# Nightmare-n/GD-MAE

Measured on AMD Instinct MI355X. Metric: MAE pre-train frames/sec (Waymo-shape, 180k pts, 75% mask), higher is better.
Workload: dtype bf16

## Files before the change

gd-mae_amd/csrc/chamfer.hip:

```cpp
#include "common.h"

struct GtParams {
  float lo[3], vs[3];
  int ncols;
  int K;
};

__global__ __launch_bounds__(256) void k_group_gt(const float* __restrict__ pts, const int* __restrict__ pt_off,
                                                  const int* __restrict__ csr, const long long* __restrict__ voxel_coords,
                                                  int M, GtParams P, float* __restrict__ gt, int* __restrict__ gidx) {
  const int lane = threadIdx.x & (GD_WAVE - 1);
  const int wib = threadIdx.x / GD_WAVE;
  for (int p = blockIdx.x * 4 + wib; p < M; p += gridDim.x * 4) {
    const int off = pt_off[p];
    const int cnt = pt_off[p + 1] - off;
    const long long* vc = voxel_coords + 4ll * p;
    const float cx = __fadd_rn(__fmul_rn(__fadd_rn((float)vc[3], 0.5f), P.vs[0]), P.lo[0]);
    const float cy = __fadd_rn(__fmul_rn(__fadd_rn((float)vc[2], 0.5f), P.vs[1]), P.lo[1]);
    const float cz = __fadd_rn(__fmul_rn(__fadd_rn((float)vc[1], 0.5f), P.vs[2]), P.lo[2]);
    for (int k = lane; k < P.K; k += GD_WAVE) {
      const int src = k < cnt ? k : k % cnt;
      const int pid = csr[off + src];
      const float* r = pts + (long long)pid * P.ncols;
      float* o = gt + ((long long)p * P.K + k) * 3;
// ... 25 lines not shown
}

template <int P1MAX>
__global__ __launch_bounds__(256) void k_chamfer(const float* __restrict__ pred, const float* __restrict__ gt,
                                                 const float* __restrict__ w, int M, int P1, int P2,
                                                 float* __restrict__ term, float* __restrict__ dpred) {
  __shared__ float sx[4][P1MAX * 3];
  const int lane = threadIdx.x & (GD_WAVE - 1);
  const int wib = threadIdx.x / GD_WAVE;
  for (int m = blockIdx.x * 4 + wib; m < M; m += gridDim.x * 4) {
    const float wm = w[m];
    float* dp = dpred + (long long)m * P1 * 3;
    if (wm == 0.f) {
      for (int e = lane; e < P1 * 3; e += GD_WAVE) dp[e] = 0.f;
      if (lane == 0) term[m] = 0.f;
      continue;
    }
    for (int e = lane; e < P1 * 3; e += GD_WAVE) sx[wib][e] = pred[(long long)m * P1 * 3 + e];
    __builtin_amdgcn_wave_barrier();
    const bool has = lane < P2;
    float y0 = 0.f, y1 = 0.f, y2 = 0.f;
    if (has) {
      const float* g = gt + ((long long)m * P2 + lane) * 3;
      y0 = g[0];
      y1 = g[1];
      y2 = g[2];
    }
    float best = INFINITY;
    int besti = 0;
    float sumx = 0.f;
    const float cx = wm / (float)P1, cy = wm / (float)P2;
    for (int i = 0; i < P1; ++i) {
      const float x0 = sx[wib][3 * i], x1 = sx[wib][3 * i + 1], x2 = sx[wib][3 * i + 2];
      const float d0 = x0 - y0, d1 = x1 - y1, d2 = x2 - y2;
      const float d = has ? (d0 * d0 + d1 * d1 + d2 * d2) : INFINITY;
      if (d < best) {
        best = d;
        besti = i;
      }
      const float dmin = gd_wave_min(d);
      const unsigned long long bal = __ballot(d == dmin);
      const int jstar = __ffsll((long long)bal) - 1;
      sumx += dmin;
      const float g0 = 2.f * cx * __shfl(d0, jstar, GD_WAVE);
      const float g1 = 2.f * cx * __shfl(d1, jstar, GD_WAVE);
      const float g2 = 2.f * cx * __shfl(d2, jstar, GD_WAVE);
      if (lane == 0) {
        dp[3 * i] = g0;
        dp[3 * i + 1] = g1;
        dp[3 * i + 2] = g2;
      }
    }
    const float sumy = gd_wave_sum(has ? best : 0.f);
    if (lane == 0) term[m] = cx * sumx + cy * sumy;
    __builtin_amdgcn_fence(__ATOMIC_RELEASE, "workgroup");
    for (int i = 0; i < P1; ++i) {
      const bool mine = has && besti == i;
      const float x0 = sx[wib][3 * i], x1 = sx[wib][3 * i + 1], x2 = sx[wib][3 * i + 2];
      const float a0 = gd_wave_sum(mine ? 2.f * cy * (x0 - y0) : 0.f);
      const float a1 = gd_wave_sum(mine ? 2.f * cy * (x1 - y1) : 0.f);
      const float a2 = gd_wave_sum(mine ? 2.f * cy * (x2 - y2) : 0.f);
      if (lane == 0) {
        dp[3 * i] += a0;
        dp[3 * i + 1] += a1;
        dp[3 * i + 2] += a2;
      }
    }
    __builtin_amdgcn_wave_barrier();
  }
}

template <int N>
__device__ __forceinline__ void ch_tstep(unsigned long long (&k)[16], int mask, int lane) {
  const bool hi = (lane & mask) != 0;
#pragma unroll
  for (int t = 0; t < N; ++t) {
    const unsigned long long send = hi ? k[t] : k[t + N];
    const unsigned long long keep = hi ? k[t + N] : k[t];
    const unsigned long long recv = __shfl_xor(send, mask, GD_WAVE);
    k[t] = keep < recv ? keep : recv;
  }
}

__global__ __launch_bounds__(256) void k_chamfer16(const float* __restrict__ pred, const float* __restrict__ gt,
                                                   const float* __restrict__ w, int M, int P2, float* __restrict__ term,
                                                   float* __restrict__ dpred) {
  __shared__ float sx[4][48];
  __shared__ float sy[4][GD_WAVE * 3];
  __shared__ int sb[4][GD_WAVE];
  __shared__ float sg[4][48];
  const int lane = threadIdx.x & (GD_WAVE - 1);
  const int wib = threadIdx.x / GD_WAVE;
  const int my_i = ((lane >> 5) & 1) * 8 + ((lane >> 4) & 1) * 4 + ((lane >> 3) & 1) * 2 + ((lane >> 2) & 1);
  for (int m = blockIdx.x * 4 + wib; m < M; m += gridDim.x * 4) {
    const float wm = w[m];
    float* dp = dpred + (long long)m * 48;
    if (wm == 0.f) {
      if (lane < 48) dp[lane] = 0.f;
      if (lane == 0) term[m] = 0.f;
      continue;
    }
    if (lane < 48) sx[wib][lane] = pred[(long long)m * 48 + lane];
    const bool has = lane < P2;
    float y0 = 0.f, y1 = 0.f, y2 = 0.f;
    if (has) {
      const float* g = gt + ((long long)m * P2 + lane) * 3;
      y0 = g[0];
      y1 = g[1];
      y2 = g[2];
    }
    __builtin_amdgcn_wave_barrier();
    const float cx = wm / 16.f, cy = wm / (float)P2;
    unsigned long long k[16];
    float best = INFINITY;
    int besti = 0;
#pragma unroll
    for (int i = 0; i < 16; ++i) {
      const float d0 = sx[wib][3 * i] - y0, d1 = sx[wib][3 * i + 1] - y1, d2 = sx[wib][3 * i + 2] - y2;
      const float d = has ? (d0 * d0 + d1 * d1 + d2 * d2) : INFINITY;
      if (d < best) {
        best = d;
        besti = i;
      }
      k[i] = ((unsigned long long)__float_as_uint(d) << 32) | (unsigned)lane;
    }
    ch_tstep<8>(k, 32, lane);
    ch_tstep<4>(k, 16, lane);
    ch_tstep<2>(k, 8, lane);
    ch_tstep<1>(k, 4, lane);
    unsigned long long k0 = k[0];
    {
      unsigned long long o = __shfl_xor(k0, 2, GD_WAVE);
      k0 = k0 < o ? k0 : o;
      o = __shfl_xor(k0, 1, GD_WAVE);
      k0 = k0 < o ? k0 : o;
    }
    const float dmin = __uint_as_float((unsigned)(k0 >> 32));
    const int jstar = (int)(k0 & 63u);
    const float ys0 = __shfl(y0, jstar, GD_WAVE), ys1 = __shfl(y1, jstar, GD_WAVE), ys2 = __shfl(y2, jstar, GD_WAVE);
    if ((lane & 3) == 0) {
      sg[wib][3 * my_i] = 2.f * cx * (sx[wib][3 * my_i] - ys0);
      sg[wib][3 * my_i + 1] = 2.f * cx * (sx[wib][3 * my_i + 1] - ys1);
      sg[wib][3 * my_i + 2] = 2.f * cx * (sx[wib][3 * my_i + 2] - ys2);
    }
    const float sumx = gd_wave_sum((lane & 3) == 0 ? dmin : 0.f);
    const float sumy = gd_wave_sum(has ? best : 0.f);
    if (lane == 0) term[m] = cx * sumx + cy * sumy;
    sy[wib][3 * lane] = y0;
    sy[wib][3 * lane + 1] = y1;
    sy[wib][3 * lane + 2] = y2;
    sb[wib][lane] = has ? besti : -1;
    __builtin_amdgcn_fence(__ATOMIC_RELEASE, "workgroup");
    __builtin_amdgcn_wave_barrier();
    if (lane < 48) {
      const int i = lane / 3, c = lane - 3 * i;
      const float xi = sx[wib][lane];
      float acc = 0.f;
      for (int j = 0; j < P2; ++j) {
        const float v = 2.f * cy * (xi - sy[wib][3 * j + c]);
        acc += sb[wib][j] == i ? v : 0.f;
      }
      dp[lane] = sg[wib][lane] + acc;
    }
    __builtin_amdgcn_wave_barrier();
  }
}

extern "C" int gdmae_chamfer(const float* pred, const float* gt, const float* weights, int M, int P1, int P2, float* term,
                             float* dpred, void* stream) {
  if (M <= 0) return 0;
  GD_REQUIRE(P2 >= 1 && P2 <= GD_WAVE, "NUM_GT_POINTS must be <= 64 (one lane per ground-truth point)");
  GD_REQUIRE(P1 >= 1 && P1 <= 64, "NUM_PRD_POINTS must be <= 64");
  int grid = gd_div_up(M, 4);
  if (grid > 8192) grid = 8192;
  if (P1 == 16)
    hipLaunchKernelGGL(k_chamfer16, dim3(grid), dim3(256), 0, (hipStream_t)stream, pred, gt, weights, M, P2, term, dpred);
  else
    hipLaunchKernelGGL((k_chamfer<64>), dim3(grid), dim3(256), 0, (hipStream_t)stream, pred, gt, weights, M, P1, P2, term,
                       dpred);
  GD_LAUNCH_CHECK();
  return 0;
}
```

gd-mae_amd/gdmae_hip/lib.py:

```python
from __future__ import annotations

import ctypes as C
import os

import torch

_HERE = os.path.dirname(os.path.abspath(__file__))
LIB_PATH = os.path.abspath(os.path.join(_HERE, "..", "csrc", "libgdmae_hip.so"))
if os.environ.get("GDMAE_LIB"):
    LIB_PATH = os.path.abspath(os.environ["GDMAE_LIB"])


class GdmaeHipError(RuntimeError):
    pass


_P, _I, _L, _F, _D, _Z = C.c_void_p, C.c_int, C.c_longlong, C.c_float, C.c_double, C.c_size_t

SIGNATURES = {
    "gdmae_abi_version": (_I, []),
    "gdmae_target_arch": (C.c_char_p, []),
    "gdmae_last_error": (C.c_char_p, []),
    "gdmae_voxelize_workspace_bytes": (_Z, [_L, _I, _I, _I, _I]),
    "gdmae_voxelize": (_I, [_P, _L, _I, _P, _P, _P, _I, _P, _P, _P, _P, _P, _P, _P, _P, _P, _P, _P, _P, _P, _P, _Z, _P]),
# ... 59 lines not shown
    "gdmae_window_attention_levels_bwd": (_I, [_P, _P, _P, _P, _P, _I, _P, _P, _P, _P, _I, _P, _P, _I, _I, _P, _F, _P, _P, _P]),
    "gdmae_conv3x3_dense_packed_bytes": (_Z, [_I, _I]),
    "gdmae_conv3x3_dense_pack": (_I, [_P, _I, _I, _I, _I, _P, _P]),
    "gdmae_conv3x3_dense": (_I, [_P, _I, _I, _I, _I, _I, _I, _P, _P, _P, _P]),
    "gdmae_conv3x3_dense_add": (_I, [_P, _I, _I, _I, _I, _I, _I, _P, _P, _P, _P, _P]),
    "gdmae_conv3x3_dense_relu": (_I, [_P, _I, _I, _I, _I, _I, _I, _P, _P, _P, _P, _P]),
    "gdmae_conv3x3_dense_stats_workspace_bytes": (_Z, [_I, _I, _I, _I]),
    "gdmae_conv3x3_dense_stat_rows": (_I, []),
    "gdmae_conv3x3_dense_stats": (_I, [_P, _I, _I, _I, _I, _I, _I, _P, _P, _P, _P, _P, _P]),
    "gdmae_bn_fold_partials": (_I, [_P, _I, _I, _D, _P, _P, _D, _D, _P, _P, _P, _P, _P, _P, _P]),
    "gdmae_conv3x3_dense_f32out": (_I, [_P, _I, _I, _I, _I, _I, _I, _P, _P, _P, _I, _P]),
    "gdmae_conv3x3_dense_dw_workspace_bytes": (_Z, [_I, _I, _I, _I, _I]),
    "gdmae_conv3x3_dense_bwd_weight": (_I, [_P, _P, _I, _I, _I, _I, _I, _I, _I, _I, _P, _P, _P]),
    "gdmae_attention_timing": (_I, [_I]),
    "gdmae_attention_timing_read": (_I, [_I, _P, _P]),
    "gdmae_kernel_timing": (_I, [_I]),
    "gdmae_kernel_timing_slots": (_I, []),
    "gdmae_kernel_timing_name": (C.c_char_p, [_I]),
    "gdmae_kernel_timing_read": (_I, [_I, _P, _P, _P, _P]),
    "gdmae_kernel_timing_read_side": (_I, [_I, _P]),
    "gdmae_add_layernorm_workspace_bytes": (_Z, [_I]),
    "gdmae_add_layernorm_fwd": (_I, [_P, _P, _I, _P, _P, _L, _I, _F, _P, _P, _P, _P]),
    "gdmae_add_layernorm_bwd": (_I, [_P, _P, _I, _P, _P, _P, _P, _I, _L, _I, _P, _P, _P, _P, _P]),
    "gdmae_prep_tokens": (_I, [_P, _P, _P, _L, _I, _P, _P, _I, _P]),
    "gdmae_sum_bf16": (_I, [_P, _I, _L, _P, _P]),
    "gdmae_add3": (_I, [_P, _P, _I, _P, _I, _L, _P, _P]),
    "gdmae_add3_to": (_I, [_P, _P, _I, _P, _I, _L, _P, _I, _P]),
    "gdmae_set_attention_impl": (_I, [_I]),
    "gdmae_sum_partials": (_I, [_P, _L, _F, _P, _I, _P]),
    "gdmae_sum_partials_gated": (_I, [_P, _L, _F, _P, _P, _F, _P]),
    "gdmae_gemm_workspace_bytes": (_Z, []),
    "gdmae_gemm_stats": (_I, [_P]),
    "gdmae_gemm_tuning": (_I, [_I]),
    "gdmae_gemm": (_I, [_P, _P, _P, _L, _L, _L, _I, _I, _I, _I, _P, _P, _P]),
    "gdmae_gemm_tn_splitk_workspace_bytes": (_Z, [_L, _I, _I]),
    "gdmae_gemm_tn_splitk": (_I, [_P, _P, _P, _L, _I, _I, _I, _I, _P, _P]),
    "gdmae_conv_block_scratch_bytes": (_Z, [_L, _L, _I, _I, _I]),
    "gdmae_spconv_packed_bytes": (_Z, [_I, _I]),
    "gdmae_spconv_pack_jobs": (_I, [_P, _I, _I, _I, _P, _P]),
    "gdmae_spconv": (_I, [_P, _I, _P, _P, _L, _I, _I, _P, _I, _P]),
    "gdmae_spconv_bias_relu": (_I, [_P, _I, _P, _P, _P, _L, _I, _I, _P, _P]),
    "gdmae_spconv_stat_rows": (_I, [_I, _I, _I]),
    "gdmae_spconv_stats": (_I, [_P, _I, _P, _P, _L, _I, _I, _P, _P, _P]),
    "gdmae_decoder_dy": (_I, [_P, _P, _I, _P, _P, _P, _P, _I, _I, _I, _P, _P]),
    "gdmae_decoder_site_rulebook": (_I, [_P, _P, _I, _L, _P, _I, _I, _P, _P]),
    "gdmae_tap_dw_rows": (_L, [_L, _I, _I]),
    "gdmae_tap_dw_workspace_bytes": (_Z, [_L, _I, _I]),
    "gdmae_tap_dw": (_I, [_P, _L, _L, _I, _P, _P, _I, _P, _I, _I, _P, _P]),
    "gdmae_decoder_block_dw_workspace_bytes": (_Z, [_L, _I]),
    "gdmae_decoder_block_dw": (_I, [_P, _P, _P, _P, _P, _L, _I, _P, _P, _I, _I, _P, _I, _I, _P, _P]),
    "gdmae_conv_block_fwd": (_I, [_P, _P]),
    "gdmae_conv_block_bwd": (_I, [_P, _P]),
    "gdmae_encoder_layer_bytes": (_I, [_L, _I, _I, _I, _I, _P, _P, _P]),
    "gdmae_dw_gemm_workspace_bytes": (_Z, [_L, _I, _I]),
    "gdmae_dw_gemm": (_I, [_P, _P, _L, _I, _I, _P, _P, _P, _P]),
    "gdmae_layer_packed_bytes": (_Z, [_I, _I]),
    "gdmae_layer_pack_jobs": (_I, [_P, _P, _P, _P, _I, _I, _P, _P]),
    "gdmae_layer_pack_job_count": (_I, [_I, _I]),
    "gdmae_tok_gemm_pack": (_I, [_P, _I, _P]),
    "gdmae_tok_gemm": (_I, [_P, _P, _P, _L, _L, _I, _I, _I, _P, _P, _P, _P, _P, _P, _F, _P, _P, _P, _P, _P, _P, _P]),
    "gdmae_tok_gemm_qkv": (_I, [_P, _P, _P, _P, _P, _L, _I, _P, _P, _P]),
    "gdmae_tok_gemm_ffn": (_I, [_P, _P, _P, _P, _P, _L, _L, _I, _P, _P, _P, _P, _F, _P, _P, _P, _P, _P, _P, _P, _P]),
    "gdmae_tok_gemm_ln_bwd_rows": (_I, [_I]),
    "gdmae_tok_gemm_ln_bwd": (_I, [_P, _P, _L, _L, _I, _I, _P, _P, _P, _P, _P, _P, _P, _P, _P, _P]),
    "gdmae_encoder_layer_fwd": (_I, [_P, _P]),
    "gdmae_encoder_layer_bwd": (_I, [_P, _P]),
    "gdmae_encoder_stage_fwd": (_I, [_P, _I, _P]),
    "gdmae_encoder_stage_bwd": (_I, [_P, _I, _P]),
    "gdmae_deconv_rows_packed_bytes": (_Z, [_I, _I, _I]),
    "gdmae_deconv_rows_pack": (_I, [_P, _I, _I, _I, _P, _P, _P]),
    "gdmae_deconv_rows_fwd": (_I, [_P, _L, _I, _I, _I, _P, _P, _P]),
    "gdmae_deconv_rows_bwd_input": (_I, [_P, _L, _I, _I, _I, _P, _P, _P]),
    "gdmae_deconv_rows_dw_workspace_bytes": (_Z, [_L, _I, _I, _I]),
    "gdmae_deconv_rows_bwd_weight": (_I, [_P, _P, _L, _I, _I, _I, _P, _P, _P]),
    "gdmae_pred_head_packed_bytes": (_Z, []),
    "gdmae_pred_head_pack": (_I, [_P, _P, _I, _I, _P, _P]),
    "gdmae_pred_head_fwd": (_I, [_P, _L, _I, _P, _P, _P, _P, _P]),
    "gdmae_pred_head_bwd_workspace_bytes": (_Z, [_L]),
    "gdmae_pred_head_bwd": (_I, [_P, _I, _P, _P, _P, _P, _L, _I, _P, _P, _P, _P, _P, _P]),
    "gdmae_encoder_set_layer_path": (_I, [_I]),
    "gdmae_encoder_stage_fused": (_I, [_P, _I]),
    "gdmae_group_gt_points": (_I, [_P, _I, _P, _P, _P, _I, _I, _P, _P, _P, _P, _P]),
    "gdmae_chamfer": (_I, [_P, _P, _P, _I, _I, _I, _P, _P, _P]),
    "gdmae_augment_collate_workspace_bytes": (_Z, [_L]),
    "gdmae_augment_collate": (_I, [_P, _L, _I, _P, _I, _P, _P, _P, _P, _P, _P]),
    "gdmae_gt_sample_workspace_bytes": (_Z, [_L]),
    "gdmae_gt_sample_select": (_I, [_P, _P, _P, _P, _I, _I, _P, _P, _P, _I, _I, _P, _P, _P, _P, _P, _P]),
    "gdmae_gt_sample_collate": (_I, [_P, _P, _I, _P, _I, _L, _I, _P, _P, _P, _P, _P, _P, _P, _P, _P, _P]),
    "gdmae_group_workspace_bytes": (_Z, [_L, _L]),
    "gdmae_ingroup_inds": (_I, [_P, _L, _L, _P, _P, _Z, _P]),
    "gdmae_group_inner_inds": (_I, [_P, _L, _L, _I, _P, _P, _Z, _P]),
    "gdmae_center_head_targets_workspace_bytes": (_Z, [_I, _I]),
    "gdmae_center_head_targets": (_I, [_P, _I, _I, _I, _P, _I, _I, _P, _P, _F, _I, _I, _I, _D, _I, _P, _P, _P, _P, _P, _P]),
    "gdmae_center_head_targets_iou": (_I, [_P, _I, _I, _I, _P, _I, _I, _P, _P, _F, _I, _I, _I, _D, _I, _P, _P, _P, _P, _P, _P, _P]),
    "gdmae_focal_loss_rows": (_I, []),
    "gdmae_focal_loss_fwd": (_I, [_P, _I, _P, _P, _I, _I, _I, _I, _P, _P, _P, _P]),
    "gdmae_focal_loss_bwd": (_I, [_P, _I, _P, _P, _I, _I, _I, _I, _P, _P, _P, _I, _P]),
    "gdmae_center_head_decode": (_I, [_P, _P, _P, _P, _P, _P, _P, _P, _I, _I, _I, _I, _P, _P, _F, _P, _F, _I, _P, _P, _P, _P, _P]),
    "gdmae_center_head_detect_workspace_bytes": (_Z, [_I, _I, _I]),
    "gdmae_center_head_detect": (_I, [_P] * 8 + [_I] * 4 + [_P, _P, _F, _P, _F, _I, _I, _P, _P, _P, _P, _P, _I, _I] + [_P] * 6),
    "gdmae_anchor_targets_workspace_bytes": (_Z, [_I, _I, _I]),
    "gdmae_anchor_targets": (_I, [_P, _I, _I, _I, _I, _I, _I, _I, _I, _P, _P, _P, _P, _P, _P, _P, _P, _P, _F, _I, _P, _P, _P, _P, _P, _P, _P]),
    "gdmae_anchor_loss_rows": (_I, []),
    "gdmae_anchor_loss_fwd": (_I, [_P, _I, _I, _I, _I, _I, _I, _I, _P, _P, _P, _P, _P, _P, _P, _P, _P]),
    "gdmae_anchor_loss_bwd": (_I, [_P, _I, _I, _I, _I, _I, _I, _I, _P, _P, _P, _P, _P, _P, _P, _P, _P]),
    "gdmae_anchor_decode": (_I, [_P, _I, _I, _I, _I, _I, _I, _I, _I, _P, _P, _P, _F, _F, _P, _P, _P]),
    "gdmae_anchor_select": (_I, [_P, _I, _I, _I, _I, _F, _P, _P, _P, _P, _P]),
    "gdmae_anchor_head_infer_packed_bytes": (_Z, [_I]),
    "gdmae_anchor_head_infer_pack": (_I, [_P, _P, _P, _P, _P, _P, _I, _I, _I, _I, _P, _P]),
    "gdmae_anchor_head_infer_workspace_bytes": (_Z, [_I, _I, _I, _I]),
    "gdmae_anchor_head_infer": (_I, [_P, _I, _I, _I, _I, _I, _I, _I, _P, _P, _P, _P, _F, _F, _F, _P, _P, _P, _P, _P, _P, _P, _P]),
    "gdmae_boxes_bev_pairs": (_I, [_P, _I, _P, _I, _I, _P, _P]),
    "gdmae_nms_workspace_bytes": (_Z, [_I]),
    "gdmae_nms_bev": (_I, [_P, _I, _F, _I, _P, _P, _P, _P]),
    "gdmae_geometry_plan_layout": (_I, [_P, _P, _I, _P, _P]),
    "gdmae_geometry_plan": (_I, [_P, _P, _P, _P, _Z, _P]),
    "gdmae_grad_sq_norm": (_I, [_P, _L, _P, _P, _P]),
    "gdmae_adam_step": (_I, [_P, _P, _P, _P, _P, _I, _F, _F, _F, _F, _F, _I, _F, _F, _P, _P]),
    "gdmae_adam_step_shadow": (_I, [_P, _P, _P, _P, _P, _I, _F, _F, _F, _F, _F, _I, _F, _F, _P, _P, _P]),
    "gdmae_roi_dfvs_pool_workspace_bytes": (_Z, [_L, _I, _I, _I, _I]),
    "gdmae_roi_dfvs_pool": (_I, [_P, _L, _I, _P, _I, _I, _I, _P, _P, _I, _I, _P, _I, _I, _I, _F, _F, _I, _I, _P, _P, _P, _P, _P, _Z, _P]),
    "gdmae_roi_graph_folded_floats": (_Z, []),
    "gdmae_roi_graph_packed_bytes": (_Z, []),
    "gdmae_roi_graph_workspace_bytes": (_Z, [_L]),
    "gdmae_roi_graph_pack": (_I, [_P, _P, _P]),
    "gdmae_roi_graph_forward": (_I, [_P, _P, _P, _I, _P, _I, _I, _I, _P, _P, _P, _P, _P, _P, _P, _Z, _P]),
}

class LayerArgs(C.Structure):
    _fields_ = ([("n", _L), ("d", _I), ("ff", _I), ("nhead", _I), ("bf16", _I), ("eps", _F), ("tau_min", _F), ("n_levels", _I),
                 ("n_win", _I * 4), ("max_tokens", _I * 4)]
                + [(k, _P) for k in ("tok_pos", "csr_tok", "win_start", "win_len", "pos_table", "Win", "bin", "Wo", "bo", "W1", "b1",
                                     "W2", "b2", "g1", "be1", "g2", "be2", "tau", "x", "y", "dy", "dx", "dWin", "dbin", "dtau", "dWo",
                                     "dbo", "dW1", "db1", "dW2", "db2", "dg1", "dbe1", "dg2", "dbe2", "saved", "scratch", "packed")]
                + [("x_bf16", _I), ("res_out", _P), ("dres", _P), ("dx_bf16", _P), ("path", _I)])


class PlanParams(C.Structure):
    _fields_ = [("n_points", _L), ("n_cols", _I), ("batch_size", _I), ("lo", _F * 3), ("vs", _F * 3), ("grid", _I * 3), ("n_stages", _I),
                ("stride", _I * 4), ("win_x", _I * 4), ("win_y", _I * 4), ("n_levels", _I * 4), ("drop_lo", (_I * 3) * 4),
                ("drop_hi", (_I * 3) * 4), ("max_tokens", (_I * 3) * 4), ("masked", _I), ("keep_frac", _D), ("n_dec", _I),
                ("dec_sources", _I * 4), ("want_pm", _I), ("cap_points", _L)]


class PlanBuffer(C.Structure):
    _fields_ = [("name", C.c_char * 40), ("offset", _L), ("bytes", _L)]


class ConvBlockArgs(C.Structure):
    _fields_ = ([("n_in", _L), ("n_out", _L), ("cin", _I), ("cout", _I), ("bf16", _I), ("x_f32", _I), ("g_f32", _I),
                 ("eps", _F), ("momentum", _F)]
                + [(k, _P) for k in ("x", "nbr", "nbr_t", "W", "gamma", "beta", "running_mean", "running_var", "num_batches", "cols",
                                     "y", "stats", "ab", "mv", "out", "g", "dx", "dW", "dgamma", "dbeta", "scratch", "packed_fwd", "packed_bwd")]
                + [("out_f32", _I)])


_lib = None


def load():
    global _lib
    if _lib is not None:
        return _lib
    if not os.path.exists(LIB_PATH):
        raise GdmaeHipError(f"{LIB_PATH} not found - build it with `python -m gdmae_hip.build` "
                            "(__graft_entry__.build()); there is no CPU fallback for the product path")
# ... 56 lines not shown
```

gd-mae_amd/gdmae_hip/ops.py:

```python
from __future__ import annotations

import torch

from . import lib as L
from . import timing

I32 = torch.int32


def _f32c(t):
    assert t.dtype == torch.float32
    return t.contiguous()


def gather_rows_raw(src: torch.Tensor, idx: torch.Tensor) -> torch.Tensor:
    src = src.contiguous()
    C = src.shape[-1]
    rb = C * src.element_size()
    out = torch.empty(tuple(idx.shape) + (C,), dtype=src.dtype, device=src.device)
    L.call("gdmae_gather_rows", L.ptr(src), L.ptr(idx.contiguous()), idx.numel(), rb, L.ptr(out), L.stream())
    return out


def scatter_rows_raw(src: torch.Tensor, idx: torch.Tensor, dst: torch.Tensor) -> torch.Tensor:
# ... 292 lines not shown
        stats = torch.empty(n, 2, dtype=torch.float32, device=a.device)
        L.call("gdmae_add_layernorm_fwd", L.ptr(a), L.ptr(b), int(b.dtype == torch.bfloat16), L.ptr(gamma.detach().contiguous()),
               L.ptr(beta.detach().contiguous()), n, d, float(eps), L.ptr(y), L.ptr(stats), None, L.stream())
        ctx.save_for_backward(a, b, gamma, stats)
        return y

    @staticmethod
    def backward(ctx, g):
        a, b, gamma, stats = ctx.saved_tensors
        n, d = a.shape
        dx = torch.empty_like(a)
        dgb = torch.empty(3 * d, dtype=torch.float32, device=a.device)
        ws = torch.empty(L.load().gdmae_add_layernorm_workspace_bytes(d), dtype=torch.uint8, device=a.device)
        L.call("gdmae_add_layernorm_bwd", L.ptr(a), L.ptr(b), int(b.dtype == torch.bfloat16), L.ptr(gamma.detach().contiguous()),
               L.ptr(stats), L.ptr(_f32c(g)), None, 0, n, d, L.ptr(dx), None, L.ptr(dgb), L.ptr(ws), L.stream())
        return dx.to(ctx.a_dtype), dx.to(b.dtype), dgb[:d], dgb[d:2 * d], None


def add_layer_norm(a, b, norm: torch.nn.LayerNorm):
    return AddLayerNorm.apply(a, b, norm.weight, norm.bias, norm.eps)


class WindowCosineAttention(torch.autograd.Function):

    @staticmethod
    def forward(ctx, qk, v, tau, wplan, nhead, tau_min):
        assert qk.dtype == v.dtype and qk.dtype in (torch.float32, torch.bfloat16)
        qk, v = qk.contiguous(), v.contiguous()
        bf = int(qk.dtype == torch.bfloat16)
        es = qk.element_size()
        n, d = v.shape
        out = torch.empty(n, d, dtype=v.dtype, device=v.device)
        tau_flat = tau.detach().reshape(1).float().contiguous()
        nl = len(wplan.n_win)
        has_lse = bool(L.load().gdmae_window_attention_levels_writes_lse(bf, nl, L.host_i32(wplan.max_tokens), d, nhead))
        lse = torch.empty(n, nhead, dtype=torch.float32, device=v.device) if has_lse else None
        with timing.kernel("k_win_attn_fwd", n * (4 * d * es + 4) + 8 * sum(wplan.n_win)):
            L.call("gdmae_window_attention_levels_fwd", L.ptr(qk), L.ptr(v), L.ptr(out), bf, L.ptr(wplan.csr_tok), L.ptr(wplan.win_start),
                   L.ptr(wplan.win_len), nl, L.host_i32(wplan.n_win), L.host_i32(wplan.max_tokens), d, nhead, L.ptr(tau_flat), float(tau_min),
                   L.ptr(lse), L.stream())
        ctx.has_lse = has_lse
        if has_lse:
            ctx.save_for_backward(qk, v, tau_flat, out, lse)
        else:
            ctx.save_for_backward(qk, v, tau_flat)
        ctx.wplan, ctx.nhead, ctx.tau_min, ctx.tau_shape, ctx.tau_dtype = wplan, nhead, tau_min, tau.shape, tau.dtype
        return out

    @staticmethod
    def backward(ctx, g):
        if ctx.has_lse:
            qk, v, tau_flat, out, lse = ctx.saved_tensors
        else:
            (qk, v, tau_flat), out, lse = ctx.saved_tensors, None, None
        wplan, H = ctx.wplan, ctx.nhead
        n, d = v.shape
        g = g.contiguous().to(v.dtype)
        bf = int(v.dtype == torch.bfloat16)
        es = v.element_size()
        dqk = torch.empty_like(qk)
        dv = torch.empty_like(v)
        n_items = [nw * H for nw in wplan.n_win]
        part = torch.zeros(max(sum(n_items), 1), dtype=torch.float32, device=v.device)
        pbase = sum(n_items)
        with timing.kernel("k_win_attn_bwd", n * (7 * d * es + 4) + 8 * sum(wplan.n_win)):
            L.call("gdmae_window_attention_levels_bwd", L.ptr(qk), L.ptr(v), L.ptr(g), L.ptr(dqk), L.ptr(dv), bf, L.ptr(part), L.ptr(wplan.csr_tok),
                   L.ptr(wplan.win_start), L.ptr(wplan.win_len), len(wplan.n_win), L.host_i32(wplan.n_win), L.host_i32(wplan.max_tokens), d, H,
                   L.ptr(tau_flat), float(ctx.tau_min), L.ptr(out), L.ptr(lse), L.stream())
        dtau = torch.empty(1, dtype=torch.float32, device=v.device)
        L.call("gdmae_sum_partials_gated", L.ptr(part), pbase, 1.0, L.ptr(dtau), L.ptr(tau_flat), float(ctx.tau_min),
               L.stream())
        return dqk, dv, dtau.view(ctx.tau_shape).to(ctx.tau_dtype), None, None, None


def group_gt_points(vox, K: int, want_index: bool = False):
    dev = vox.points.device
    gt = torch.empty(vox.M, K, 3, dtype=torch.float32, device=dev)
    gi = torch.empty(vox.M, K, dtype=I32, device=dev) if want_index else None
    L.call("gdmae_group_gt_points", L.ptr(vox.points), vox.n_cols, L.ptr(vox.pt_off), L.ptr(vox.pillar_pts),
           L.ptr(vox.voxel_coords), vox.M, K, L.host_f32(vox.lo), L.host_f32(vox.vs), L.ptr(gt), L.ptr(gi), L.stream())
    return (gt, gi) if want_index else gt


LAZY_SCALE = {}


class ChamferLoss(torch.autograd.Function):

    @staticmethod
    def forward(ctx, pred, gt, weights, lazy_scale=False):
        ctx.pred_dtype = pred.dtype
        ctx.lazy = bool(lazy_scale and pred.dtype == torch.float32)
        pred, gt, weights = _f32c(pred.float()), _f32c(gt), _f32c(weights)
        M, P1, _ = pred.shape
        P2 = gt.shape[1]
        term = torch.empty(max(M, 1), dtype=torch.float32, device=pred.device)
        dpred = torch.empty_like(pred)
        L.call("gdmae_chamfer", L.ptr(pred), L.ptr(gt), L.ptr(weights), M, P1, P2, L.ptr(term), L.ptr(dpred), L.stream())
        res = torch.empty(2, dtype=torch.float32, device=pred.device)
        L.call("gdmae_weighted_mean_finish", L.ptr(term), L.ptr(weights), M, L.ptr(res), L.stream())
        ctx.save_for_backward(dpred, res)
        return res[0]

    @staticmethod
    def backward(ctx, g):
        dpred, res = ctx.saved_tensors
        inv = res[1]
        if ctx.lazy:
            LAZY_SCALE.clear()
            LAZY_SCALE[dpred.data_ptr()] = (g.detach().reshape(1).float().contiguous(), res[1:2])
            return dpred, None, None, None
        if ctx.pred_dtype == torch.float32:
            return dpred * (g * inv), None, None, None
        out = torch.empty_like(dpred, dtype=ctx.pred_dtype)
        torch.mul(dpred, g * inv, out=out)
        return out, None, None, None
```

gd-mae_amd/pcdet/models/backbones_3d/spt_backbone_mae.py:

```python
import torch
import torch.nn as nn

from .spt_backbone import SSTBlockV1, build_decoder, run_decoder, stage_plan_args
from ...utils.spconv_utils import SparseConvTensor
from gdmae_hip import decoder as gdec, ops, plan as gplan


def _only_the_pred_head_sees_the_gradient(pred) -> bool:
    fn = pred.grad_fn
    if fn is None or not type(fn).__name__.startswith('ViewBackward') or pred._backward_hooks or pred.retains_grad:
        return False
    nxt = [f for f, _ in fn.next_functions if f is not None]
    if len(nxt) != 1 or 'PredHeadFn' not in type(nxt[0]).__name__:
        return False
    return not getattr(nxt[0], '_tensor_pre_hooks', None) and not getattr(nxt[0], '_pre_hooks', None) and not getattr(nxt[0], '_retains_grad_hooks', None)


class _DeferredPlan:
    __slots__ = ("_mod", "_args", "_pf")

    def __init__(self, mod, args):
        self._mod, self._args, self._pf = mod, args, None

    def __call__(self):
        if self._pf is None and self._args is not None:
            points, batch_size, noise, ready = self._args
            self._args = None
            self._pf = self._mod.prefetch_plan(points, batch_size, noise=noise, ready=ready)

    def ensure_issued(self):
        if self._mod is not None and getattr(self._mod, '_pre_conv_hook', None) is self:
            self._mod._pre_conv_hook = None
        self()

    def finish(self):
        self.ensure_issued()
        pf, self._pf, self._mod = self._pf, None, None
        return pf.finish()


class SPTBackboneMAE(nn.Module):
    decoder_impl = 'sparse'
    dense_spatial_features = True
    decoder_conv_impl = 'tiles'

    def __init__(self, model_cfg, input_channels, grid_size, voxel_size, point_cloud_range, **kwargs):
        super().__init__()
        self.model_cfg, self.grid_size, self.voxel_size, self.point_cloud_range = model_cfg, grid_size, voxel_size, point_cloud_range
        self.sparse_shape = grid_size[[1, 0]]
        self.mask_cfg = model_cfg.get('MASK_CONFIG', None)
        self.mask_ratio = self.mask_cfg.RATIO if self.mask_cfg is not None else 0.0
        c = input_channels
        self.sst_blocks = nn.ModuleList()
        for b in model_cfg.SST_BLOCK_LIST:
            self.sst_blocks.append(SSTBlockV1(b, c, b.NAME))
            c = b.ENCODER.D_MODEL
        self.decoder_deblocks, self.decoder_conv_out, c = build_decoder(model_cfg)
        self.decoder_pred = nn.Linear(c, self.mask_cfg.NUM_PRD_POINTS * 3, bias=True)
        self.forward_ret_dict = {}
        self.num_point_features = c

    def get_loss(self, tb_dict=None):
        tb_dict = {} if tb_dict is None else tb_dict
        r = self.forward_ret_dict
        pred = r['pred_points']
        lazy = bool(r.get('pred_lazy_scale', False)) and _only_the_pred_head_sees_the_gradient(pred)
        return ops.ChamferLoss.apply(pred, r['gt_points'], r['mask'], lazy), tb_dict

    def forward(self, batch_dict):
        vox = batch_dict['_gdmae_vox']
        all_feat, all_coords = batch_dict['voxel_features'], batch_dict['voxel_coords']
        ep = batch_dict.get('_gdmae_plan', None)
        if ep is None:
            ep = gplan.encoder_plan(vox, *stage_plan_args(self.model_cfg.SST_BLOCK_LIST),
                                    keep_frac=1 - self.mask_ratio, noise=batch_dict.get('mae_noise', None),
                                    dec_sources=self._dec_sources())
        batch_dict['voxel_mae_mask'] = ep.mask
        batch_dict['_gdmae_plan'] = ep
        x = SparseConvTensor(ops.GatherUnique.apply(all_feat, ep.tok_pillar), ep, 0)
        sync = batch_dict.get('_gdmae_grad_sync', None)
        hidden = []
        for i, blk in enumerate(self.sst_blocks):
            if sync is not None:
                sync.mark(x.features, [f'backbone_3d.sst_blocks.{i}'])
            x = blk(x)
            hidden.append(x)
        if sync is not None:
            sync.mark(x.features, ['backbone_3d.decoder'])
        feats, strides = {}, {}
        Y0 = int(self.sparse_shape[0])
        for i, h in enumerate(hidden):
            feats[f'x_conv{i + 1}'] = h
            strides[f'x_conv{i + 1}'] = Y0 // h.spatial_shape[0]
        B, X, Y = int(batch_dict['batch_size']), int(self.grid_size[0]), int(self.grid_size[1])
        if self.decoder_impl == 'sparse' and self.training:
            hook, self._pre_conv_hook = getattr(self, '_pre_conv_hook', None), None
            pyramid, sf = gdec.sparse_decoder(self.model_cfg, self.decoder_deblocks, self.decoder_conv_out, hidden,
                                              vox.pillar_cell, vox.cell2pillar, B, Y, X,
                                              want_dense=self.dense_spatial_features, conv_impl=self.decoder_conv_impl,
                                              pre_conv_hook=hook)
        else:
            sf = run_decoder(self.model_cfg, self.decoder_deblocks, self.decoder_conv_out, hidden)
            assert sf.shape[0] == B and sf.shape[2] == Y and sf.shape[3] == X
            pyramid = ops.GatherUnique.apply(sf.permute(0, 2, 3, 1).reshape(B * Y * X, sf.shape[1]), vox.pillar_cell)
        src0 = self.model_cfg.FEATURES_SOURCE[0]
        batch_dict.update({'encoded_spconv_tensor': hidden[-1], 'encoded_spconv_tensor_stride': Y0 // hidden[-1].spatial_shape[0],
                           'multi_scale_3d_features': feats, 'multi_scale_3d_strides': strides, 'spatial_features': sf,
                           'spatial_features_stride': strides[src0] // self.model_cfg.FUSE_LAYER[src0].UPSAMPLE_STRIDE})
        batch_dict.update({'voxel_features': pyramid, 'voxel_coords': all_coords,
                           'voxel_shuffle_inds': torch.arange(all_coords.shape[0], device=all_coords.device)})
        self.forward_ret_dict = self.target_assigner(batch_dict)
        return batch_dict

    def prefetch_plan(self, points, batch_size, noise=None, ready=None):
        return gplan.PlanPrefetch(points, self.point_cloud_range, self.voxel_size, self.grid_size, int(batch_size),
                                  *stage_plan_args(self.model_cfg.SST_BLOCK_LIST), keep_frac=1 - self.mask_ratio, noise=noise,
                                  ready=ready, dec_sources=self._dec_sources())

    def prefetch_plan_under_decoder(self, points, batch_size, noise=None, ready=None):
        self._pre_conv_hook = d = _DeferredPlan(self, (points, batch_size, noise, ready))
        return d

    def _dec_sources(self):
        if self.decoder_impl != 'sparse' or self.decoder_conv_impl != 'tiles':
            return None
        return [int(src[-1]) - 1 for src in self.model_cfg.FEATURES_SOURCE]

    def target_assigner(self, batch_dict):
        vox = batch_dict['_gdmae_vox']
        gt = ops.group_gt_points(vox, self.mask_cfg.NUM_GT_POINTS)
        flat = gdec.pred_head(batch_dict['voxel_features'], self.decoder_pred)
        return {'pred_points': flat.view(vox.M, -1, 3), 'gt_points': gt, 'mask': batch_dict['voxel_mae_mask'],
                'pred_lazy_scale': bool(getattr(flat, '_gd_pred_head', False))}
```

include/gdmae_hip.h:

```cpp
#ifndef GDMAE_HIP_H
#define GDMAE_HIP_H

#include <stddef.h>
#include <stdint.h>

#ifdef __cplusplus
extern "C" {
#endif

int gdmae_abi_version(void);
const char* gdmae_target_arch(void);
const char* gdmae_last_error(void);

size_t gdmae_voxelize_workspace_bytes(long long n_points, int batch_size, int gx, int gy, int gz);
int gdmae_voxelize(const float* points, long long n_points, int n_cols, const float* lo, const float* vs,
                   const int* grid_xyz, int batch_size, float* points_out, long long* point_coords,
                   long long* inverse, int* inverse32, long long* voxel_coords, int* pillar_cell,
                   int* pillar_pt_off, int* pillar_pts, int* point_rank, int* sample_pillar_off,
                   float* pillar_mean, int* cell2pillar, int* counts, void* workspace, size_t workspace_bytes,
                   void* stream);

int gdmae_decorate_points(const float* points, const long long* point_coords, const int* inverse32,
                          const float* pillar_mean, long long N, int n_cols, const float* lo, const float* vs,
                          float* out, void* stream);
// ... 256 lines not shown
  float* dx;
  float *dWin, *dbin, *dtau, *dWo, *dbo, *dW1, *db1, *dW2, *db2, *dg1, *dbe1, *dg2, *dbe2;
  void* saved;
  void* scratch;
  const void* packed;
  int x_bf16;
  void* res_out;
  const void* dres;
  void* dx_bf16;
  int path;
} gdmae_layer_args;
size_t gdmae_layer_packed_bytes(int d, int ff);
int gdmae_layer_pack_jobs(const float* Win, const float* Wo, const float* W1, const float* W2, int d, int ff, void* packed,
                          long long* jobs_host );
int gdmae_layer_pack_job_count(int d, int ff);
int gdmae_tok_gemm_pack(const long long* jobs_dev, int n_jobs, void* stream);
int gdmae_tok_gemm(const void* X, const void* Wp, const void* bias, long long n, long long n_pad, int K, int N, int epilogue,
                   void* out0, void* out1, const void* aux, const float* res, const float* gamma, const float* beta, float eps,
                   float* y, float* stats, void* y_bf16, const float* pos_table, const int* tok_pos, void* ypos_bf16,
                   void* stream);

int gdmae_tok_gemm_qkv(const void* Xpos, const void* X, const void* Wp_qk, const void* Wp_v, const void* bias3, long long n_pad,
                       int d, void* qk, void* v, void* stream);

int gdmae_tok_gemm_ffn(const void* X, const void* W1p, const void* b1, const void* W2p, const void* b2, long long n, long long n_pad,
                       int d, void* h, const float* res, const float* gamma, const float* beta, float eps, float* y, float* stats,
                       void* y_bf16, const float* pos_table, const int* tok_pos, void* ypos_bf16, void* f_out, void* stream);

int gdmae_tok_gemm_ln_bwd_rows(int N);
int gdmae_tok_gemm_ln_bwd(const void* X, const void* Wp, long long n, long long n_pad, int K, int N, const float* dy,
                          const void* dy2_bf16, const float* ln_a, const void* ln_b_bf16, const float* stats,
                          const float* gamma, float* dx, void* dx_bf16, float* part, void* stream);
int gdmae_encoder_layer_bytes(long long n, int d, int ff, int nhead, int bf16, size_t* saved_bytes,
                              size_t* fwd_scratch_bytes, size_t* bwd_scratch_bytes);
int gdmae_encoder_layer_fwd(const gdmae_layer_args* args , void* stream);
int gdmae_encoder_layer_bwd(const gdmae_layer_args* args , void* stream);
int gdmae_encoder_stage_fwd(const gdmae_layer_args* layers , int n_layers, void* stream);
int gdmae_encoder_stage_bwd(const gdmae_layer_args* layers , int n_layers, void* stream);
int gdmae_encoder_set_layer_path(int path);
int gdmae_encoder_stage_fused(const gdmae_layer_args* layers , int n_layers);

size_t gdmae_deconv_rows_packed_bytes(int cin, int cout, int s);
int gdmae_deconv_rows_pack(const float* weight, int cin, int cout, int s, void* packed_fwd, void* packed_bwd, void* stream);
int gdmae_deconv_rows_fwd(const void* X, long long n, int cin, int cout, int s, const void* packed_fwd, void* P, void* stream);
int gdmae_deconv_rows_bwd_input(const void* dP, long long n, int cin, int cout, int s, const void* packed_bwd, void* dX, void* stream);
size_t gdmae_deconv_rows_dw_workspace_bytes(long long n, int cin, int cout, int s);
int gdmae_deconv_rows_bwd_weight(const void* X, const void* dP, long long n, int cin, int cout, int s, float* dW, void* workspace,
                                 void* stream);

size_t gdmae_pred_head_packed_bytes(void);
int gdmae_pred_head_pack(const float* weight, const float* bias, int n_in, int n_out, void* packed, void* stream);
int gdmae_pred_head_fwd(const float* X, long long n, int n_out, const void* packed, void* Y, void* X_bf16 , float* Y_f32 ,
                        void* stream);
size_t gdmae_pred_head_bwd_workspace_bytes(long long n);
int gdmae_pred_head_bwd(const void* dY, int dy_f32 ,
                        void* dY_bf16 ,
                        const float* scale_a, const float* scale_b ,
                        const void* X_bf16, long long n, int n_out,
                        const void* packed, float* dX, float* dW, float* db, void* workspace, void* stream);

size_t gdmae_conv3x3_dense_packed_bytes(int cin, int cout);
int gdmae_conv3x3_dense_pack(const float* weight, int cin, int cout, int dil, int transposed, void* packed, void* stream);
int gdmae_conv3x3_dense(const void* X, int B, int H, int W, int cin_l, int cout_l, int dil, const void* packed, const float* bias,
                        void* Y, void* stream);
int gdmae_conv3x3_dense_add(const void* X, int B, int H, int W, int cin_l, int cout_l, int dil, const void* packed, const float* bias,
                            const void* addend, void* Y, void* stream);
int gdmae_conv3x3_dense_relu(const void* X, int B, int H, int W, int cin_l, int cout_l, int dil, const void* packed, const float* bias,
                             const void* shortcut, void* Y, void* stream);
size_t gdmae_conv3x3_dense_stats_workspace_bytes(int B, int H, int W, int cout_l);
int gdmae_conv3x3_dense_stat_rows(void);
int gdmae_conv3x3_dense_stats(const void* X, int B, int H, int W, int cin_l, int cout_l, int dil, const void* packed, const float* bias,
                              void* Y, float* stat_rows, void* workspace, void* stream);
int gdmae_conv3x3_dense_f32out(const void* X, int B, int H, int W, int cin_l, int cout_l, int dil, const void* packed, const float* bias,
                               float* Y, int accumulate, void* stream);
size_t gdmae_conv3x3_dense_dw_workspace_bytes(int B, int H, int W, int cin_l, int cout_l);
int gdmae_conv3x3_dense_bwd_weight(const void* X, const void* dY, int B, int H, int W, int cin_l, int cout_l, int cin, int cout, int dil,
                                   float* dW, void* workspace, void* stream);

int gdmae_group_gt_points(const float* points, int n_cols, const int* pillar_pt_off, const int* pillar_pts,
                          const long long* voxel_coords, int M, int K, const float* lo, const float* vs,
                          float* gt_points, int* gt_index, void* stream);
int gdmae_chamfer(const float* pred, const float* gt, const float* weights, int M, int P1, int P2, float* term,
                  float* dpred, void* stream);

size_t gdmae_augment_collate_workspace_bytes(long long n_raw);
int gdmae_augment_collate(const float* raw, long long n_raw, int F, const int* frame_off, int B, const float* frame_params,
                          const float* xy_range , float* out, int* kept_off, void* workspace, void* stream);

size_t gdmae_gt_sample_workspace_bytes(long long n_rows);
int gdmae_gt_sample_select(const float* boxes, const int* frame_desc_host, const int* frame_desc, const int* cand_group, int B,
                           int n_groups, const float* frame_params, const float* range ,
                           const float* extra_width , int min_corners, int cap, int* valid, float* rm_boxes,
                           int* n_valid, float* gt_boxes, int* num_gt, void* stream);
int gdmae_gt_sample_collate(const float* raw, const float* db, int F, const int* seg, int S, long long n_rows, int B,
                            const float* frame_params, const float* boxes, const int* valid, const float* rm_boxes,
                            const int* n_valid, const float* xy_range , float* out, int* kept_off, void* workspace,
                            void* stream);

size_t gdmae_group_workspace_bytes(long long n, long long n_groups);
int gdmae_ingroup_inds(const long long* group_inds, long long n, long long n_groups, long long* out_inds,
                       void* workspace, size_t workspace_bytes, void* stream);
int gdmae_group_inner_inds(const long long* inverse_inds, long long n, long long M, int K, long long* group_inds,
                           void* workspace, size_t workspace_bytes, void* stream);

#define GDMAE_PLAN_MAX_STAGES 4
typedef struct gdmae_plan_params {
  long long n_points;
  int n_cols, batch_size;
  float lo[3], vs[3];
  int grid[3];
  int n_stages;
  int stride[GDMAE_PLAN_MAX_STAGES];
  int win_x[GDMAE_PLAN_MAX_STAGES], win_y[GDMAE_PLAN_MAX_STAGES];
  int n_levels[GDMAE_PLAN_MAX_STAGES];
  int drop_lo[GDMAE_PLAN_MAX_STAGES][3], drop_hi[GDMAE_PLAN_MAX_STAGES][3], max_tokens[GDMAE_PLAN_MAX_STAGES][3];
  int masked;
  double keep_frac;
  int n_dec;
  int dec_sources[GDMAE_PLAN_MAX_STAGES];
  int want_pm;
  long long cap_points;
} gdmae_plan_params;
typedef struct gdmae_plan_buffer {
  char name[40];
  long long offset, bytes;
} gdmae_plan_buffer;
int gdmae_geometry_plan_layout(const gdmae_plan_params* p, gdmae_plan_buffer* table, int max_entries, int* n_entries,
                               size_t* total_bytes);
int gdmae_geometry_plan(const gdmae_plan_params* p, const float* points, const float* noise, void* arena, size_t arena_bytes,
                        void* stream);

size_t gdmae_center_head_targets_workspace_bytes(int B, int num_max_objs);
int gdmae_center_head_targets(const float* gt_boxes, int B, int n_max, int box_dim, const int* class_map, int n_class_total,
                              int n_cls, const float* pc_range , const float* voxel_size ,
                              float feature_map_stride, int fw, int fh, int num_max_objs, double gaussian_overlap, int min_radius,
                              float* heatmap, float* ret_boxes, long long* inds, long long* mask, void* workspace, void* stream);
int gdmae_focal_loss_rows(void);
int gdmae_focal_loss_fwd(const void* logits, int logits_bf16, const long long* strides_byxc, const float* gt, int B, int C, int H, int W,
                         float* prob, float* partials, float* out4, void* stream);
int gdmae_focal_loss_bwd(const void* logits, int logits_bf16, const long long* strides_byxc, const float* gt, int B, int C, int H, int W,
                         const float* out4, const float* grad_out, void* dlogits, int dlogits_bf16, void* stream);
int gdmae_center_head_targets_iou(const float* gt_boxes, int B, int n_max, int box_dim, const int* class_map, int n_class_total,
                                  int n_cls, const float* pc_range, const float* voxel_size, float feature_map_stride, int fw, int fh,
                                  int num_max_objs, double gaussian_overlap, int min_radius, float* heatmap, float* ret_boxes,
                                  float* iou_boxes, long long* inds, long long* mask, void* workspace, void* stream);
int gdmae_center_head_decode(const long long* cell, const float* score, const float* center, const float* center_z,
                             const float* dim, const float* rot, const float* vel, const float* iou, int B, int K, int H, int W,
                             const float* pc_range , const float* voxel_size ,
                             float feature_map_stride, const float* post_center_limit_range , float score_thresh,
                             int use_score_thresh, float* boxes, int* labels, float* ious, unsigned char* valid, void* stream);
size_t gdmae_center_head_detect_workspace_bytes(int B, int K, int box_dim);
int gdmae_center_head_detect(const long long* cell, const float* score, const float* center, const float* center_z, const float* dim,
                             const float* rot, const float* vel, const float* iou, int B, int K, int H, int W, const float* pc_range,
                             const float* voxel_size, float feature_map_stride, const float* post_center_limit_range, float score_thresh,
                             int use_score_thresh, int C, const float* thresh, const int* pre_max, const int* post_max,
                             const float* rectifier, const int* to_global, int class_aware, int n_out, float* boxes, float* scores,
                             long long* labels, int* count, void* workspace, void* stream);

int gdmae_boxes_bev_pairs(const float* boxes_a, int n, const float* boxes_b, int m, int mode, float* out, void* stream);
size_t gdmae_nms_workspace_bytes(int n);
int gdmae_nms_bev(const float* boxes, int n, float thresh, int rotated, long long* keep, int* n_keep, void* workspace,
                  void* stream);

size_t gdmae_anchor_targets_workspace_bytes(int B, int n_cls, int n_max);
int gdmae_anchor_targets(const float* gt_boxes, int B, int n_max, int box_dim, int H, int W, int K, int n_cls, int n_names,
                         const int* name_idx, const int* slot_cls, const float* xr, const float* yr, const float* xc, const float* yc,
// ... 53 lines not shown
```

Before: 1093.

## Fuse ground-truth point grouping into the chamfer kernel via lazy pillar targets

The chamfer loss kernel now reads ground-truth points straight from the pillar-major point array, using pillar offsets and voxel centres. This removes the separate group_gt kernel launch and the M×K×3 intermediate buffer it wrote. A lazy PillarTargets object and a dict subclass build the grouped tensor only if something else asks for gt_points. Template specialisation adds a compile-time full-wave path for K=64. Masked pillars now skip all ground-truth loads, and the fused path assumes contiguous float32 pillar-major points.

Measured after the change: 1103 (median of 6 runs). About the same (+0.9%).

```diff
diff --git a/gd-mae_amd/csrc/chamfer.hip b/gd-mae_amd/csrc/chamfer.hip
--- a/gd-mae_amd/csrc/chamfer.hip
+++ b/gd-mae_amd/csrc/chamfer.hip
@@ -131,28 +131,48 @@
   }
 }
 
+template <bool PILLARS, bool FULL>
 __global__ __launch_bounds__(256) void k_chamfer16(const float* __restrict__ pred, const float* __restrict__ gt,
-                                                   const float* __restrict__ w, int M, int P2, float* __restrict__ term,
-                                                   float* __restrict__ dpred) {
+                                                   const int* __restrict__ pt_off, const long long* __restrict__ voxel_coords,
+                                                   GtParams P, const float* __restrict__ w, int M, int P2,
+                                                   float* __restrict__ term, float* __restrict__ dpred) {
   __shared__ float sx[4][48];
   __shared__ float sy[4][GD_WAVE * 3];
   __shared__ int sb[4][GD_WAVE];
   __shared__ float sg[4][48];
   const int lane = threadIdx.x & (GD_WAVE - 1);
-  const int wib = threadIdx.x / GD_WAVE;
+  const int wib = __builtin_amdgcn_readfirstlane(threadIdx.x / GD_WAVE);
+  const int col_i = lane / 3, col_c = lane - 3 * col_i;
   const int my_i = ((lane >> 5) & 1) * 8 + ((lane >> 4) & 1) * 4 + ((lane >> 3) & 1) * 2 + ((lane >> 2) & 1);
   for (int m = blockIdx.x * 4 + wib; m < M; m += gridDim.x * 4) {
     const float wm = w[m];
     float* dp = dpred + (long long)m * 48;
-    if (wm == 0.f) {
+    int off = 0, cnt = 1;
+    if (PILLARS) {
+      off = pt_off[m];
+      cnt = pt_off[m + 1] - off;
+    }
+    if (wm == 0.f || cnt <= 0) {
       if (lane < 48) dp[lane] = 0.f;
       if (lane == 0) term[m] = 0.f;
       continue;
     }
     if (lane < 48) sx[wib][lane] = pred[(long long)m * 48 + lane];
-    const bool has = lane < P2;
+    const bool has = FULL || lane < P2;
     float y0 = 0.f, y1 = 0.f, y2 = 0.f;
-    if (has) {
+    if (PILLARS) {
+      const long long* vc = voxel_coords + 4ll * m;
+      const float ctr0 = __fadd_rn(__fmul_rn(__fadd_rn((float)vc[3], 0.5f), P.vs[0]), P.lo[0]);
+      const float ctr1 = __fadd_rn(__fmul_rn(__fadd_rn((float)vc[2], 0.5f), P.vs[1]), P.lo[1]);
+      const float ctr2 = __fadd_rn(__fmul_rn(__fadd_rn((float)vc[1], 0.5f), P.vs[2]), P.lo[2]);
+      if (has) {
+        const int src = lane < cnt ? lane : lane % cnt;
+        const float* r = gt + (long long)(off + src) * P.ncols;
+        y0 = __fsub_rn(r[1], ctr0);
+        y1 = __fsub_rn(r[2], ctr1);
+        y2 = __fsub_rn(r[3], ctr2);
+      }
+    } else if (has) {
       const float* g = gt + ((long long)m * P2 + lane) * 3;
       y0 = g[0];
       y1 = g[1];
@@ -202,12 +222,11 @@
     __builtin_amdgcn_fence(__ATOMIC_RELEASE, "workgroup");
     __builtin_amdgcn_wave_barrier();
     if (lane < 48) {
-      const int i = lane / 3, c = lane - 3 * i;
       const float xi = sx[wib][lane];
       float acc = 0.f;
-      for (int j = 0; j < P2; ++j) {
-        const float v = 2.f * cy * (xi - sy[wib][3 * j + c]);
-        acc += sb[wib][j] == i ? v : 0.f;
+      for (int j = 0; j < (FULL ? GD_WAVE : P2); ++j) {
+        const float v = 2.f * cy * (xi - sy[wib][3 * j + col_c]);
+        acc += sb[wib][j] == col_i ? v : 0.f;
       }
       dp[lane] = sg[wib][lane] + acc;
     }
@@ -222,11 +241,41 @@
   GD_REQUIRE(P1 >= 1 && P1 <= 64, "NUM_PRD_POINTS must be <= 64");
   int grid = gd_div_up(M, 4);
   if (grid > 8192) grid = 8192;
-  if (P1 == 16)
-    hipLaunchKernelGGL(k_chamfer16, dim3(grid), dim3(256), 0, (hipStream_t)stream, pred, gt, weights, M, P2, term, dpred);
+  if (P1 == 16 && P2 == GD_WAVE)
+    hipLaunchKernelGGL((k_chamfer16<false, true>), dim3(grid), dim3(256), 0, (hipStream_t)stream, pred, gt, (const int*)nullptr,
+                       (const long long*)nullptr, GtParams{}, weights, M, P2, term, dpred);
+  else if (P1 == 16)
+    hipLaunchKernelGGL((k_chamfer16<false, false>), dim3(grid), dim3(256), 0, (hipStream_t)stream, pred, gt, (const int*)nullptr,
+                       (const long long*)nullptr, GtParams{}, weights, M, P2, term, dpred);
   else
     hipLaunchKernelGGL((k_chamfer<64>), dim3(grid), dim3(256), 0, (hipStream_t)stream, pred, gt, weights, M, P1, P2, term,
                        dpred);
   GD_LAUNCH_CHECK();
   return 0;
 }
+
+extern "C" int gdmae_chamfer_pillars(const float* pred, const float* points_pm, int n_cols, const int* pillar_pt_off,
+                                     const long long* voxel_coords, const float* lo, const float* vs, int K,
+                                     const float* weights, int M, int P1, float* term, float* dpred, void* stream) {
+  GD_REQUIRE(P1 == 16, "gdmae_chamfer_pillars: NUM_PRD_POINTS must be 16 (gdmae_group_gt_points + gdmae_chamfer otherwise)");
+  GD_REQUIRE(K >= 1 && K <= GD_WAVE, "NUM_GT_POINTS must be 1 .. 64 (one lane per ground-truth point)");
+  GD_REQUIRE(n_cols >= 4, "point rows are (batch, x, y, z, ...)");
+  if (M <= 0) return 0;
+  GtParams P;
+  for (int i = 0; i < 3; ++i) {
+    P.lo[i] = lo[i];
+    P.vs[i] = vs[i];
+  }
+  P.ncols = n_cols;
+  P.K = K;
+  int grid = gd_div_up(M, 4);
+  if (grid > 8192) grid = 8192;
+  if (K == GD_WAVE)
+    hipLaunchKernelGGL((k_chamfer16<true, true>), dim3(grid), dim3(256), 0, (hipStream_t)stream, pred, points_pm, pillar_pt_off,
+                       voxel_coords, P, weights, M, K, term, dpred);
+  else
+    hipLaunchKernelGGL((k_chamfer16<true, false>), dim3(grid), dim3(256), 0, (hipStream_t)stream, pred, points_pm, pillar_pt_off,
+                       voxel_coords, P, weights, M, K, term, dpred);
+  GD_LAUNCH_CHECK();
+  return 0;
+}
diff --git a/gd-mae_amd/gdmae_hip/lib.py b/gd-mae_amd/gdmae_hip/lib.py
--- a/gd-mae_amd/gdmae_hip/lib.py
+++ b/gd-mae_amd/gdmae_hip/lib.py
@@ -165,6 +165,7 @@
     "gdmae_encoder_stage_fused": (_I, [_P, _I]),
     "gdmae_group_gt_points": (_I, [_P, _I, _P, _P, _P, _I, _I, _P, _P, _P, _P, _P]),
     "gdmae_chamfer": (_I, [_P, _P, _P, _I, _I, _I, _P, _P, _P]),
+    "gdmae_chamfer_pillars": (_I, [_P, _P, _I, _P, _P, _P, _P, _I, _P, _I, _I, _P, _P, _P]),
     "gdmae_augment_collate_workspace_bytes": (_Z, [_L]),
     "gdmae_augment_collate": (_I, [_P, _L, _I, _P, _I, _P, _P, _P, _P, _P, _P]),
     "gdmae_gt_sample_workspace_bytes": (_Z, [_L]),
diff --git a/gd-mae_amd/gdmae_hip/ops.py b/gd-mae_amd/gdmae_hip/ops.py
--- a/gd-mae_amd/gdmae_hip/ops.py
+++ b/gd-mae_amd/gdmae_hip/ops.py
@@ -398,6 +398,21 @@
     return (gt, gi) if want_index else gt
 
 
+class PillarTargets:
+    __slots__ = ("vox", "K")
+
+    def __init__(self, vox, K: int):
+        self.vox, self.K = vox, int(K)
+
+    def materialize(self) -> torch.Tensor:
+        return group_gt_points(self.vox, self.K)
+
+    def loads_from_pillars(self, P1: int) -> bool:
+        pm = self.vox.points_pm
+        return (P1 == 16 and 1 <= self.K <= 64 and pm is not None and pm.dtype == torch.float32 and pm.is_contiguous()
+                and pm.shape[1] == self.vox.n_cols >= 4)
+
+
 LAZY_SCALE = {}
 
 
@@ -407,12 +422,18 @@
     def forward(ctx, pred, gt, weights, lazy_scale=False):
         ctx.pred_dtype = pred.dtype
         ctx.lazy = bool(lazy_scale and pred.dtype == torch.float32)
-        pred, gt, weights = _f32c(pred.float()), _f32c(gt), _f32c(weights)
+        pred, weights = _f32c(pred.float()), _f32c(weights)
         M, P1, _ = pred.shape
-        P2 = gt.shape[1]
         term = torch.empty(max(M, 1), dtype=torch.float32, device=pred.device)
         dpred = torch.empty_like(pred)
-        L.call("gdmae_chamfer", L.ptr(pred), L.ptr(gt), L.ptr(weights), M, P1, P2, L.ptr(term), L.ptr(dpred), L.stream())
+        if isinstance(gt, PillarTargets) and gt.loads_from_pillars(P1):
+            vox = gt.vox
+            assert vox.M == M
+            L.call("gdmae_chamfer_pillars", L.ptr(pred), L.ptr(vox.points_pm), vox.n_cols, L.ptr(vox.pt_off), L.ptr(vox.voxel_coords),
+                   L.host_f32(vox.lo), L.host_f32(vox.vs), gt.K, L.ptr(weights), M, P1, L.ptr(term), L.ptr(dpred), L.stream())
+        else:
+            gt = _f32c(gt.materialize() if isinstance(gt, PillarTargets) else gt)
+            L.call("gdmae_chamfer", L.ptr(pred), L.ptr(gt), L.ptr(weights), M, P1, gt.shape[1], L.ptr(term), L.ptr(dpred), L.stream())
         res = torch.empty(2, dtype=torch.float32, device=pred.device)
         L.call("gdmae_weighted_mean_finish", L.ptr(term), L.ptr(weights), M, L.ptr(res), L.stream())
         ctx.save_for_backward(dpred, res)
diff --git a/gd-mae_amd/pcdet/models/backbones_3d/spt_backbone_mae.py b/gd-mae_amd/pcdet/models/backbones_3d/spt_backbone_mae.py
--- a/gd-mae_amd/pcdet/models/backbones_3d/spt_backbone_mae.py
+++ b/gd-mae_amd/pcdet/models/backbones_3d/spt_backbone_mae.py
@@ -39,6 +39,15 @@
         return pf.finish()
 
 
+class _TargetDict(dict):
+
+    def __missing__(self, key):
+        if key != 'gt_points' or 'gt_targets' not in self:
+            raise KeyError(key)
+        gt = self[key] = self['gt_targets'].materialize()
+        return gt
+
+
 class SPTBackboneMAE(nn.Module):
     decoder_impl = 'sparse'
     dense_spatial_features = True
@@ -65,7 +74,8 @@
         r = self.forward_ret_dict
         pred = r['pred_points']
         lazy = bool(r.get('pred_lazy_scale', False)) and _only_the_pred_head_sees_the_gradient(pred)
-        return ops.ChamferLoss.apply(pred, r['gt_points'], r['mask'], lazy), tb_dict
+        gt = r['gt_points'] if 'gt_points' in r else r['gt_targets']
+        return ops.ChamferLoss.apply(pred, gt, r['mask'], lazy), tb_dict
 
     def forward(self, batch_dict):
         vox = batch_dict['_gdmae_vox']
@@ -128,7 +138,7 @@
 
     def target_assigner(self, batch_dict):
         vox = batch_dict['_gdmae_vox']
-        gt = ops.group_gt_points(vox, self.mask_cfg.NUM_GT_POINTS)
+        gt = ops.PillarTargets(vox, self.mask_cfg.NUM_GT_POINTS)
         flat = gdec.pred_head(batch_dict['voxel_features'], self.decoder_pred)
-        return {'pred_points': flat.view(vox.M, -1, 3), 'gt_points': gt, 'mask': batch_dict['voxel_mae_mask'],
-                'pred_lazy_scale': bool(getattr(flat, '_gd_pred_head', False))}
+        return _TargetDict({'pred_points': flat.view(vox.M, -1, 3), 'gt_targets': gt, 'mask': batch_dict['voxel_mae_mask'],
+                            'pred_lazy_scale': bool(getattr(flat, '_gd_pred_head', False))})
diff --git a/include/gdmae_hip.h b/include/gdmae_hip.h
--- a/include/gdmae_hip.h
+++ b/include/gdmae_hip.h
@@ -362,6 +362,9 @@
                           float* gt_points, int* gt_index, void* stream);
 int gdmae_chamfer(const float* pred, const float* gt, const float* weights, int M, int P1, int P2, float* term,
                   float* dpred, void* stream);
+int gdmae_chamfer_pillars(const float* pred, const float* points_pm, int n_cols, const int* pillar_pt_off,
+                          const long long* voxel_coords, const float* lo, const float* vs, int K,
+                          const float* weights, int M, int P1, float* term, float* dpred, void* stream);
 
 size_t gdmae_augment_collate_workspace_bytes(long long n_raw);
 int gdmae_augment_collate(const float* raw, long long n_raw, int F, const int* frame_off, int B, const float* frame_params,
```
